# ltinphan/convex-mpc-unitree-go2

Measured on AMD Instinct MI355X. Metric: batched QP solves/sec (N=16, 4-leg friction cone) at 1/2/4/8 MI355X, higher is better.
Workload: dtype f32

## Files before the change

### convex-mpc-unitree-go2_amd/cmpc/_lib.py

```python
from __future__ import annotations

import ctypes
import os
from pathlib import Path

from .build import LIB

ABI_VERSION = 6
ABI_COMPAT = (5, 6) if os.environ.get("CMPC_ALLOW_ABI5") == "1" else (6,)
NUM_STATS = 4
CMPC_OK = 0


class CParams(ctypes.Structure):
    _fields_ = [
        ("abi_version", ctypes.c_int32),
        ("N", ctypes.c_int32),
        ("Q", ctypes.c_float * 12),
        ("R", ctypes.c_float * 12),
        ("mu", ctypes.c_float),
        ("fz_min", ctypes.c_float),
        ("eps_abs", ctypes.c_float),
        ("eps_rel", ctypes.c_float),
        ("max_iter", ctypes.c_int32),
# ... 5 lines not shown
        ("polish_refine", ctypes.c_int32),
        ("polish_tol", ctypes.c_float),
        ("polish_repairs", ctypes.c_int32),
        ("reserved0", ctypes.c_int32),
        ("check_termination", ctypes.c_int32),
        ("max_batch", ctypes.c_int64),
    ]


def _io_fields(*names):
    head = ("Ad", "Bd", "gd", "x0", "xref", "contact", "mu", "fz_min")
    values = dict(face_tol=ctypes.c_float, prim_tol=ctypes.c_float, dual_tol=ctypes.c_float,
                  max_rounds=ctypes.c_int32)
    return ([("size", ctypes.c_uint32)] +
            [(n, values.get(n, ctypes.c_void_p)) for n in head + names])


class CSolveIO(ctypes.Structure):
    _fields_ = _io_fields("w_init", "y_init", "lam_init", "w_out", "y_out", "lam_out", "status",
                          "iters", "Q", "R")


class CKktIO(ctypes.Structure):
    _fields_ = _io_fields("Q", "R", "w", "lam", "face_tol", "res")


class CGainIO(ctypes.Structure):
    _fields_ = _io_fields("Q", "R", "w", "faces", "face_tol", "K", "Vx", "Vxx", "u_star",
                          "faces_out")


class CVjpIO(ctypes.Structure):
    _fields_ = _io_fields("Q", "R", "w", "faces", "face_tol", "gw", "g_x0", "g_xref", "g_gd", "g_Q",
                          "g_R", "g_mu", "g_fz_min", "g_Ad", "g_Bd")


class CRefineIO(ctypes.Structure):
    _fields_ = _io_fields("Q", "R", "w", "faces", "face_tol", "max_rounds", "prim_tol", "dual_tol",
                          "info", "res", "w64", "lam_out", "faces_out", "w_out", "status")


REFINE_INVALID, REFINE_ROUNDS, REFINE_CYCLE, REFINE_MAX_ROUNDS = -1, -2, -3, 16
REFINE_OUTPUTS = ("info", "res", "w64", "lam", "faces")

FACE_FZ_MIN, FACE_FX_POS, FACE_FX_NEG, FACE_FY_POS, FACE_FY_NEG = 1, 2, 4, 8, 16
GAIN_OUTPUTS = ("K", "Vx", "Vxx", "u_star", "faces")
VJP_OUTPUTS = ("x0", "xref", "gd", "Q", "R", "mu", "fz_min", "Ad", "Bd")

KKT_COLUMNS = ("cost", "stat", "prim", "comp")

EXPORTS = ("cmpc_params_default", "cmpc_plan_create", "cmpc_solve", "cmpc_plan_destroy",
           "cmpc_build_dynamics", "cmpc_solve_warm", "cmpc_solve_ref", "cmpc_solve_io_run", "cmpc_kkt_run", "cmpc_gain_run", "cmpc_vjp_run", "cmpc_refine_run", "cmpc_generate_traj", "cmpc_leg_torque", "cmpc_srb_step",
           "cmpc_plan_set_timing", "cmpc_plan_timing_read", "cmpc_plan_set_team", "cmpc_plan_team_batch",
           "cmpc_plan_set_heavy_first",
           "cmpc_plan_heavy_first_batch", "cmpc_plan_solve_kernel", "cmpc_plan_stats",
           "cmpc_last_error", "cmpc_version")
NUM_BINS = 5
BIN_CAPS = (96, 128, 144, 160, 192)
NUM_SOLVE_KERNELS = 3
KERNEL_BINS = ((1, 0), (3, 2), (4,))
KERNEL_NAMES = ("solve_group_kernel<128, 96>", "solve_group_kernel<160, 144>",
                "solve_group_kernel<192, 0>")

_lib = None


def load(path: str | Path | None = None) -> ctypes.CDLL:
    global _lib
    if _lib is not None and path is None:
        return _lib
    if path is None and os.environ.get("CMPC_LIB"):
        path = os.environ["CMPC_LIB"]
    p = Path(path) if path is not None else LIB
    if not p.exists():
        raise RuntimeError(f"cmpc: HIP library {p} not built (run __graft_entry__.build() or "
                           f"python -m cmpc.build); there is no CPU fallback")
    lib = ctypes.CDLL(str(p))
    vp = ctypes.c_void_p
    lib.cmpc_params_default.argtypes = [ctypes.POINTER(CParams)]
    lib.cmpc_params_default.restype = None
    lib.cmpc_plan_create.argtypes = [ctypes.POINTER(CParams), ctypes.POINTER(vp)]
    lib.cmpc_plan_create.restype = ctypes.c_int
    lib.cmpc_solve.argtypes = [vp, ctypes.c_int64] + [vp] * 10
    lib.cmpc_solve.restype = ctypes.c_int
    if hasattr(lib, "cmpc_solve_warm"):
        lib.cmpc_solve_warm.argtypes = [vp, ctypes.c_int64] + [vp] * 13
        lib.cmpc_solve_warm.restype = ctypes.c_int
    if hasattr(lib, "cmpc_solve_ref"):
        lib.cmpc_solve_ref.argtypes = [vp, ctypes.c_int64] + [vp] * 13
        lib.cmpc_solve_ref.restype = ctypes.c_int
    if hasattr(lib, "cmpc_solve_io_run"):
        lib.cmpc_solve_io_run.argtypes = [vp, ctypes.c_int64, ctypes.POINTER(CSolveIO), vp]
        lib.cmpc_solve_io_run.restype = ctypes.c_int
    if hasattr(lib, "cmpc_kkt_run"):
        lib.cmpc_kkt_run.argtypes = [vp, ctypes.c_int64, ctypes.POINTER(CKktIO), vp]
        lib.cmpc_kkt_run.restype = ctypes.c_int
    if hasattr(lib, "cmpc_gain_run"):
        lib.cmpc_gain_run.argtypes = [vp, ctypes.c_int64, ctypes.POINTER(CGainIO), vp]
        lib.cmpc_gain_run.restype = ctypes.c_int
    if hasattr(lib, "cmpc_vjp_run"):
        lib.cmpc_vjp_run.argtypes = [vp, ctypes.c_int64, ctypes.POINTER(CVjpIO), vp]
        lib.cmpc_vjp_run.restype = ctypes.c_int
    if hasattr(lib, "cmpc_refine_run"):
        lib.cmpc_refine_run.argtypes = [vp, ctypes.c_int64, ctypes.POINTER(CRefineIO), vp]
        lib.cmpc_refine_run.restype = ctypes.c_int
    lib.cmpc_build_dynamics.argtypes = [vp, ctypes.c_int64, ctypes.c_float] + [vp] * 8
    lib.cmpc_build_dynamics.restype = ctypes.c_int
    if hasattr(lib, "cmpc_generate_traj"):
        lib.cmpc_generate_traj.argtypes = [vp, ctypes.c_int64, ctypes.c_double] + [vp] * 11
        lib.cmpc_generate_traj.restype = ctypes.c_int
    if hasattr(lib, "cmpc_leg_torque"):
        lib.cmpc_leg_torque.argtypes = ([vp, ctypes.c_int64, vp, vp, vp, ctypes.c_int64] +
                                        [vp] * 12 + [ctypes.c_double, vp, vp])
        lib.cmpc_leg_torque.restype = ctypes.c_int
    if hasattr(lib, "cmpc_srb_step"):
        lib.cmpc_srb_step.argtypes = ([vp, ctypes.c_int64, ctypes.c_int, ctypes.c_double] + [vp] * 5 +
                                      [ctypes.c_int64] + [vp] * 5)
        lib.cmpc_srb_step.restype = ctypes.c_int
    lib.cmpc_plan_destroy.argtypes = [vp]
    lib.cmpc_plan_destroy.restype = None
    lib.cmpc_plan_set_timing.argtypes = [vp, ctypes.c_int]
    lib.cmpc_plan_set_timing.restype = ctypes.c_int
    lib.cmpc_plan_timing_read.argtypes = [vp, ctypes.POINTER(ctypes.c_float),
                                          ctypes.POINTER(ctypes.c_int32)]
    lib.cmpc_plan_timing_read.restype = ctypes.c_int
    if hasattr(lib, "cmpc_plan_set_team"):
        lib.cmpc_plan_set_team.argtypes = [vp, ctypes.c_int64]
        lib.cmpc_plan_set_team.restype = ctypes.c_int
        lib.cmpc_plan_team_batch.argtypes = [vp, ctypes.POINTER(ctypes.c_int64)]
        lib.cmpc_plan_team_batch.restype = ctypes.c_int
    if hasattr(lib, "cmpc_plan_set_heavy_first"):
        lib.cmpc_plan_set_heavy_first.argtypes = [vp, ctypes.c_int64]
        lib.cmpc_plan_set_heavy_first.restype = ctypes.c_int
        lib.cmpc_plan_heavy_first_batch.argtypes = [vp, ctypes.POINTER(ctypes.c_int64)]
        lib.cmpc_plan_heavy_first_batch.restype = ctypes.c_int
    if hasattr(lib, "cmpc_plan_stats"):
        lib.cmpc_plan_stats.argtypes = [vp, ctypes.POINTER(ctypes.c_uint64), ctypes.c_int]
        lib.cmpc_plan_stats.restype = ctypes.c_int
    if hasattr(lib, "cmpc_plan_solve_kernel"):
        lib.cmpc_plan_solve_kernel.argtypes = [vp, ctypes.c_int64, ctypes.c_int]
        lib.cmpc_plan_solve_kernel.restype = ctypes.c_char_p
    lib.cmpc_last_error.argtypes = []
    lib.cmpc_last_error.restype = ctypes.c_char_p
    lib.cmpc_version.argtypes = []
    lib.cmpc_version.restype = ctypes.c_char_p
    if path is None:
        _lib = lib
    return lib


def last_error(lib=None) -> str:
    lib = lib or load()
    return lib.cmpc_last_error().decode()
```

### convex-mpc-unitree-go2_amd/cmpc/solver.py

```python
from __future__ import annotations

import ctypes
from dataclasses import dataclass, field, fields
from typing import Optional

import torch

from . import _lib

STATUS_STRINGS = {1: "solved", 2: "solved inaccurate", -2: "maximum iterations reached",
                  -10: "unsolved"}
KKT_COLUMNS = _lib.KKT_COLUMNS


@dataclass
class SolverParams:
    N: int = 16
    Q: tuple = (1, 1, 50, 10, 20, 1, 2, 2, 1, 1, 1, 1)
    R: tuple = (1e-5,) * 12
    mu: float = 0.8
    fz_min: float = 10.0
    eps_abs: float = 1e-4
    eps_rel: float = 1e-4
    max_iter: int = 1000
# ... 97 lines not shown
            self._h = None

    def __del__(self):
        try:
            self.close()
        except Exception:
            pass

    def _same_device(self, t: torch.Tensor):
        if t.device != self.device:
            raise ValueError(f"cmpc: tensors are on {t.device} but the plan was created on "
                             f"{self.device}")

    def _fill_io(self, io, required: dict, optional: dict):
        for spec, skip_none in ((required, False), (optional, True)):
            for name, (t, dtype, shape) in spec.items():
                if t is None and skip_none:
                    continue
                _dev_tensor(t, name, dtype, shape)
                self._same_device(t)
                setattr(io, name, t.data_ptr())

    def _need(self, entry: str, method: str):
        if not hasattr(self.lib, entry):
            raise CmpcError(f"cmpc: this libcmpc.so has no {entry}: Plan.{method} needs a library "
                            "built from sources that declare it")

    def _results(self, io, spec: dict, want, always, out, device) -> dict:
        out = dict(out or {})
        res = {}
        for name in tuple(always) + tuple(n for n in want if n not in always):
            field, dtype, shape = spec[name]
            t = out.get(name)
            if t is None:
                t = torch.empty(shape, dtype=dtype, device=device)
            _dev_tensor(t, name, dtype, shape)
            self._same_device(t)
            setattr(io, field, t.data_ptr())
            res[name] = t
        return res

    def set_timing(self, enable: bool):
        _check(self.lib, self.lib.cmpc_plan_set_timing(self._h, int(bool(enable))),
               "cmpc_plan_set_timing")

    def set_team(self, max_batch: int):
        _check(self.lib, self.lib.cmpc_plan_set_team(self._h, int(max_batch)),
               "cmpc_plan_set_team")

    def team_batch(self) -> int:
        v = ctypes.c_int64()
        _check(self.lib, self.lib.cmpc_plan_team_batch(self._h, ctypes.byref(v)),
               "cmpc_plan_team_batch")
        return int(v.value)

    def set_heavy_first(self, min_batch: int):
        _check(self.lib, self.lib.cmpc_plan_set_heavy_first(self._h, int(min_batch)),
               "cmpc_plan_set_heavy_first")

    def heavy_first_batch(self) -> int:
        v = ctypes.c_int64()
        _check(self.lib, self.lib.cmpc_plan_heavy_first_batch(self._h, ctypes.byref(v)),
               "cmpc_plan_heavy_first_batch")
        return int(v.value)

    def solve_kernels(self, B: int) -> list:
        if not hasattr(self.lib, "cmpc_plan_solve_kernel"):
            return [None] * _lib.NUM_SOLVE_KERNELS
        out = []
        for k in range(_lib.NUM_SOLVE_KERNELS):
            r = self.lib.cmpc_plan_solve_kernel(self._h, int(B), k)
            out.append(r.decode() if r else None)
        return out

    def stats(self, reset: bool = False) -> dict:
        keys = ("loose", "status2_cert", "guard_refactors", "reserved")
        if not hasattr(self.lib, "cmpc_plan_stats"):
            return {k: None for k in keys[:3]}
        v = (ctypes.c_uint64 * _lib.NUM_STATS)()
        _check(self.lib, self.lib.cmpc_plan_stats(self._h, v, int(bool(reset))), "cmpc_plan_stats")
        return {k: int(x) for k, x in zip(keys[:3], list(v))}

    def timing_read(self):
        ms = (ctypes.c_float * 4)()
        calls = (ctypes.c_int32 * 4)()
        _check(self.lib, self.lib.cmpc_plan_timing_read(self._h, ms, calls),
               "cmpc_plan_timing_read")
        k = _lib.NUM_SOLVE_KERNELS
        return list(ms)[:k], list(calls)[:k]

    def solve(self, Ad, Bd, gd, x0, xref, contact, out=None, stream=None, w_init=None,
              y_init=None, y_out=None, lam_init=None, lam_out=None, mu=None, fz_min=None,
              Q=None, R=None):
        N = self.params.N
        B = Ad.shape[0]
        f32 = torch.float32
        for name, spec in _problem_spec(B, N, Ad, Bd, gd, x0, xref, contact).items():
            _dev_tensor(spec[0], name, *spec[1:])
        self._same_device(Ad)
        for t in (Bd, gd, x0, xref, contact):
            if t.device != Ad.device:
                raise ValueError("all inputs must be on the same device")
        if out is None:
            w = torch.empty((B, 24 * N), dtype=f32, device=Ad.device)
            status = torch.empty((B,), dtype=torch.int32, device=Ad.device)
            iters = torch.empty((B,), dtype=torch.int32, device=Ad.device)
# ... 334 lines not shown
```

### convex-mpc-unitree-go2_amd/csrc/cmpc_device.h

```cpp
#pragma once
#include <stdint.h>

namespace cmpc {

struct KParams {
  int N;
  float Q2[12];
  float R2[12];
  float mu, fz_min;
  float rho0, sigma, alpha;
  float eps_abs, eps_rel;
  float polish_tol;
  float r2_min;
  int max_iter;
  int adaptive_interval;
  int polish_stable;
  int polish_refine;
  int polish_repairs;
  int check_every;
  int latency_mode;
};

struct Inputs {
  const float* Ad = nullptr;
  const float* Bd = nullptr;
  const float* gd = nullptr;
  const float* x0 = nullptr;
  const float* xref = nullptr;
  const uint8_t* contact = nullptr;
  const float* w_init = nullptr;
  const float* y_init = nullptr;
  const float* lam_init = nullptr;
  const float* mu = nullptr;
  const float* fz_min = nullptr;
  const float* Q = nullptr;
  const float* R = nullptr;
};
struct Outputs {
  float* w = nullptr;
  int32_t* status = nullptr;
  int32_t* iters = nullptr;
  float* y = nullptr;
  float* lam = nullptr;
  unsigned long long* stats = nullptr;
};

constexpr int kNumBins = 5;
constexpr int kBinCap[kNumBins] = {96, 128, 144, 160, 192};

}
```

### convex-mpc-unitree-go2_amd/csrc/cmpc_host.hip

```cpp
#include <hip/hip_runtime.h>
#include <stddef.h>
#include <stdlib.h>
#include <stdint.h>
#include <stdio.h>
#include <string.h>

#include <algorithm>
#include <cmath>
#include <string>
#include <vector>

#include "cmpc.h"
#include "cmpc_device.h"

#include "cmpc_wave.hip"
#include "cmpc_dynamics.hip"
#include "cmpc_traj.hip"
#include "cmpc_leg.hip"
#include "cmpc_sim.hip"
#include "cmpc_kkt.hip"
#include "cmpc_gain.hip"
#include "cmpc_vjp.hip"
#include "cmpc_refine.hip"

// ... 170 lines not shown
  p->max_batch = 65536;
}

int cmpc_plan_create(const cmpc_params* p, cmpc_plan** out) {
  if (!p || !out) return fail(CMPC_E_INVALID, "cmpc_plan_create: null argument");
  *out = nullptr;
  if (p->abi_version != CMPC_ABI_VERSION)
    return fail(CMPC_E_INVALID, "cmpc_plan_create: abi_version mismatch");
  if (p->N < 1 || p->N > 16) return fail(CMPC_E_INVALID, "cmpc_plan_create: N must be in 1..16");
  for (int i = 0; i < 12; ++i) {
    if (!(p->Q[i] >= 0.f) || !std::isfinite(p->Q[i]))
      return fail(CMPC_E_INVALID, "cmpc_plan_create: Q must be finite and >= 0");
    if (!(p->R[i] > 0.f) || !std::isfinite(p->R[i]))
      return fail(CMPC_E_INVALID, "cmpc_plan_create: R must be finite and > 0");
  }
  if (!(p->mu > 0.f) || !std::isfinite(p->mu)) return fail(CMPC_E_INVALID, "cmpc_plan_create: mu must be > 0");
  if (!std::isfinite(p->fz_min)) return fail(CMPC_E_INVALID, "cmpc_plan_create: fz_min must be finite");
  if (p->max_iter < 1) return fail(CMPC_E_INVALID, "cmpc_plan_create: max_iter must be >= 1");
  if (!(p->rho > 0.f) || !(p->sigma >= 0.f) || !(p->alpha > 0.f && p->alpha < 2.f))
    return fail(CMPC_E_INVALID, "cmpc_plan_create: need rho > 0, sigma >= 0, 0 < alpha < 2");
  if (p->polish_stable < 1 || p->polish_refine < 1 || !(p->polish_tol > 0.f) ||
      p->polish_repairs < 0 || p->check_termination < 1)
    return fail(CMPC_E_INVALID, "cmpc_plan_create: polish settings out of range");
  if (p->adaptive_rho_interval < 0 || p->max_batch < 1 || p->max_batch > (1LL << 30))
    return fail(CMPC_E_INVALID, "cmpc_plan_create: adaptive_rho_interval/max_batch out of range");
  if (p->reserved0 != 0)
    return fail(CMPC_E_INVALID, "cmpc_plan_create: reserved0 must be 0 (ABI 4's ipm_facts: the "
                                "interior-point fallback was removed)");

  cmpc_plan* pl = new cmpc_plan();
  pl->p = *p;
  cmpc::KParams& k = pl->kp;
  k.N = p->N;
  k.r2_min = 2.f * p->R[0];
  for (int i = 0; i < 12; ++i) {
    k.Q2[i] = 2.f * p->Q[i];
    k.R2[i] = 2.f * p->R[i];
    k.r2_min = std::min(k.r2_min, k.R2[i]);
  }
  k.mu = p->mu;
  k.fz_min = p->fz_min;
  k.rho0 = p->rho;
  k.sigma = p->sigma;
  k.alpha = p->alpha;
  k.eps_abs = p->eps_abs;
  k.eps_rel = p->eps_rel;
  k.polish_tol = p->polish_tol;
  k.max_iter = p->max_iter;
  k.adaptive_interval = p->adaptive_rho_interval;
  k.polish_stable = p->polish_stable;
  k.polish_refine = p->polish_refine;
  k.polish_repairs = p->polish_repairs;
  k.check_every = p->check_termination;

  hipError_t e = hipGetDevice(&pl->device);
  if (e != hipSuccess) { delete pl; return hip_fail(e, "hipGetDevice"); }
  int cus = 0;
  e = hipDeviceGetAttribute(&cus, hipDeviceAttributeMultiprocessorCount, pl->device);
  pl->cus = cus;
  if (e != hipSuccess) { delete pl; return hip_fail(e, "hipDeviceGetAttribute"); }
  size_t work_floats = 0;
  for (int k = 0; k < kNumGroups; ++k) {
    int nb = 0;
    e = hipOccupancyMaxActiveBlocksPerMultiprocessor(&nb, group_fn(k), 64, 0);
    if (e != hipSuccess) { delete pl; return hip_fail(e, "hipOccupancyMaxActiveBlocksPerMultiprocessor"); }
    if (nb < 1) { delete pl; return fail(CMPC_E_HIP, "cmpc_plan_create: solve kernel cannot be resident"); }
#ifdef CMPC_STAMPS
    if (const char* cap = getenv("CMPC_BLOCKS_PER_CU")) {
      const int c = atoi(cap);
      if (c >= 1 && c < nb) nb = c;
    }
#endif
    pl->grid[k] = nb * cus;
    pl->slab[k] = group_slab(k);
    pl->work_off[k] = work_floats;
    work_floats += (size_t)pl->grid[k] * pl->slab[k];
  }
  {
    int nb = 0;
    e = hipOccupancyMaxActiveBlocksPerMultiprocessor(&nb, cmpc::solve_team_kernel<kTeamWaves, 2>,
                                                     64 * kTeamWaves, 0);
    if (e != hipSuccess) { delete pl; return hip_fail(e, "hipOccupancyMaxActiveBlocksPerMultiprocessor"); }
    if (nb < 1) nb = 1;
    pl->team_grid = nb * cus;
    e = hipOccupancyMaxActiveBlocksPerMultiprocessor(&nb, cmpc::solve_team_kernel<kTeamWaves, 1>,
                                                     64 * kTeamWaves, 0);
    if (e != hipSuccess) { delete pl; return hip_fail(e, "hipOccupancyMaxActiveBlocksPerMultiprocessor"); }
    pl->team_grid1 = nb < 1 ? 0 : cus;
    pl->team_slab = std::max({cmpc::TeamCfg<192, kTeamWaves>::SLAB, cmpc::TeamCfg<160, kTeamWaves>::SLAB,
                              cmpc::TeamCfg<128, kTeamWaves>::SLAB, cmpc::TeamCfg<96, kTeamWaves>::SLAB});
    work_floats = std::max(work_floats, (size_t)pl->team_grid * pl->team_slab);
  }
  e = hipMalloc(&pl->d_counters, 2 * cmpc::kNumBins * sizeof(int));
  if (e != hipSuccess) { delete pl; return fail(CMPC_E_NOMEM, "hipMalloc counters failed"); }
  e = hipMalloc(&pl->d_work, work_floats * sizeof(float));
  if (e != hipSuccess) {
    (void)hipFree(pl->d_counters);
    delete pl;
    return fail(CMPC_E_NOMEM, "hipMalloc workspace failed");
  }
  e = hipMalloc(&pl->d_lists, (size_t)cmpc::kNumBins * p->max_batch * sizeof(int));
  if (e != hipSuccess) {
    (void)hipFree(pl->d_counters);
    (void)hipFree(pl->d_work);
    delete pl;
    return fail(CMPC_E_NOMEM, "hipMalloc lists failed");
// ... 372 lines not shown
  if (B == 0) return CMPC_OK;
  if (!t || !gait || !force || !J_foot || !J_full || !M || !C || !g || !dq || !Jdot_dq ||
      !foot_pos || !foot_vel || !body || !hip || !state || !tau)
    return fail(CMPC_E_INVALID, "cmpc_leg_torque: null array argument");
  cmpc::LegArgs a{t, gait, force, force_stride, J_foot, J_full, M, C, g, dq, Jdot_dq, foot_pos,
                  foot_vel, body, hip, state, tau_max, tau};
  hipLaunchKernelGGL(cmpc::leg_kernel, dim3(grid_stride_blocks(B, 16384)), dim3(64), 0,
                     (hipStream_t)stream, B, a);
  hipError_t e = hipGetLastError();
  if (e != hipSuccess) return hip_fail(e, "leg_kernel launch");
  return CMPC_OK;
}

int cmpc_srb_step(cmpc_plan* pl, int64_t B, int nsub, double dt, const double* t_now,
                  const double* gait, const float* mass, const float* inertia_body,
                  const float* force, int64_t force_stride, const float* hip, float* x,
                  float* feet, uint8_t* contact_state, void* stream) {
  if (!pl) return fail(CMPC_E_INVALID, "cmpc_srb_step: null plan");
  if (int rc = check_device(pl, "cmpc_srb_step")) return rc;
  if (B < 0 || nsub < 0) return fail(CMPC_E_INVALID, "cmpc_srb_step: negative batch or nsub");
  if (!(dt > 0.0) || !std::isfinite(dt)) return fail(CMPC_E_INVALID, "cmpc_srb_step: dt must be > 0");
  if (force_stride < 12) return fail(CMPC_E_INVALID, "cmpc_srb_step: force_stride must be >= 12");
  if (B == 0 || nsub == 0) return CMPC_OK;
  if (!t_now || !gait || !mass || !inertia_body || !force || !hip || !x || !feet || !contact_state)
    return fail(CMPC_E_INVALID, "cmpc_srb_step: null array argument");
  const unsigned blocks = (unsigned)((B + 255) / 256);
  hipLaunchKernelGGL(cmpc::srb_kernel, dim3(blocks), dim3(256), 0, (hipStream_t)stream, B, nsub,
                     dt, t_now, gait, mass, inertia_body, force, force_stride, hip, x, feet,
                     contact_state);
  hipError_t e = hipGetLastError();
  if (e != hipSuccess) return hip_fail(e, "srb_kernel launch");
  return CMPC_OK;
}

int cmpc_plan_set_timing(cmpc_plan* pl, int enable) {
  if (!pl) return fail(CMPC_E_INVALID, "cmpc_plan_set_timing: null plan");
  pl->timing = enable != 0;
  return CMPC_OK;
}

int cmpc_plan_set_team(cmpc_plan* pl, int64_t max_batch) {
  if (!pl) return fail(CMPC_E_INVALID, "cmpc_plan_set_team: null plan");
  if (max_batch < -1) return fail(CMPC_E_INVALID, "cmpc_plan_set_team: max_batch must be >= -1");
  pl->team_max_batch = max_batch;
  return CMPC_OK;
}

int cmpc_plan_team_batch(const cmpc_plan* pl, int64_t* max_batch) {
  if (!pl || !max_batch) return fail(CMPC_E_INVALID, "cmpc_plan_team_batch: null argument");
  *max_batch = team_batch(pl);
  return CMPC_OK;
}

int cmpc_plan_set_heavy_first(cmpc_plan* pl, int64_t min_batch) {
  if (!pl) return fail(CMPC_E_INVALID, "cmpc_plan_set_heavy_first: null plan");
  if (min_batch < -1) return fail(CMPC_E_INVALID, "cmpc_plan_set_heavy_first: min_batch must be >= -1");
  pl->heavy_first_min_batch = min_batch;
  return CMPC_OK;
}

int cmpc_plan_heavy_first_batch(const cmpc_plan* pl, int64_t* min_batch) {
  if (!pl || !min_batch) return fail(CMPC_E_INVALID, "cmpc_plan_heavy_first_batch: null argument");
  *min_batch = heavy_first_batch(pl);
  return CMPC_OK;
}

const char* cmpc_plan_solve_kernel(const cmpc_plan* pl, int64_t B, int k) {
  if (!pl || B < 1 || k < 0 || k >= kNumGroups) return nullptr;
  if (B <= team_batch(pl))
    return k != 0 ? nullptr : team_one_per_cu(pl, B) ? "solve_team_kernel<4, 1>" : "solve_team_kernel<4, 2>";
  if (!has_group(pl, k)) return nullptr;
  return group_name(k);
}

int cmpc_plan_timing_read(cmpc_plan* pl, float* ms_per_kernel, int32_t* calls_per_kernel) {
  if (!pl || !ms_per_kernel || !calls_per_kernel)
    return fail(CMPC_E_INVALID, "cmpc_plan_timing_read: null argument");
  for (int k = 0; k < kNumGroups; ++k) { ms_per_kernel[k] = 0.f; calls_per_kernel[k] = 0; }
  for (auto& r : pl->recs) {
    hipError_t e = hipEventSynchronize(r.b);
    if (e != hipSuccess) return hip_fail(e, "hipEventSynchronize");
    float ms = 0.f;
    e = hipEventElapsedTime(&ms, r.a, r.b);
    if (e != hipSuccess) return hip_fail(e, "hipEventElapsedTime");
    ms_per_kernel[r.group] += ms;
    calls_per_kernel[r.group] += 1;
    pl->pool.push_back(r);
  }
  pl->recs.clear();
  return CMPC_OK;
}

void cmpc_plan_destroy(cmpc_plan* pl) {
  if (!pl) return;
  for (auto& r : pl->recs) { (void)hipEventDestroy(r.a); (void)hipEventDestroy(r.b); }
  for (auto& r : pl->pool) { (void)hipEventDestroy(r.a); (void)hipEventDestroy(r.b); }
  if (pl->side) (void)hipStreamDestroy(pl->side);
  if (pl->top) (void)hipStreamDestroy(pl->top);
  if (pl->fork) (void)hipEventDestroy(pl->fork);
  if (pl->join) (void)hipEventDestroy(pl->join);
  if (pl->join_top) (void)hipEventDestroy(pl->join_top);
  (void)hipFree(pl->d_counters);
  (void)hipFree(pl->d_lists);
  (void)hipFree(pl->d_work);
  if (pl->d_stats) (void)hipFree(pl->d_stats);
  delete pl;
// ... 33 lines not shown
```

### convex-mpc-unitree-go2_amd/csrc/cmpc_solve.h

```cpp
#pragma once
#include "cmpc_team.hip"

#include "cmpc_condense.h"
#include "cmpc_factor.h"
#include "cmpc_gradient.h"
#include "cmpc_polish.h"

namespace cmpc {

template <int NC>
__device__ __forceinline__ int session_start(Smem<NC>& s, const KParams& P, int ntri, int nfail,
                                             int& ntried, bool& seen) {
  const int l = opaque_lane();
  WSYNC();
  uint8_t c = 0;
  if (l < ntri) {
    c = (uint8_t)s.code[l];
    s.tpat[0][l] = c;
  }
  ntried = 1;
  seen = false;
#pragma unroll
  for (int k = 0; k < kFailMem; ++k) {
    if (k >= nfail) break;
    const bool diff = (l < ntri) && (s.fpat[k][l] != c);
    seen |= (__any(diff) == 0);
  }
  if (seen) return 0;
  return (nfail >= 2) ? min(P.polish_repairs, kLateRepairs) : P.polish_repairs;
}

template <int NC>
__device__ __forceinline__ bool tried_before(Smem<NC>& s, int ntri, int ntried) {
  const int l = opaque_lane();
  WSYNC();
  const uint8_t c = (l < ntri) ? (uint8_t)s.tcnt[l] : 0;
  bool hit = false;
  for (int k = 0; k < ntried; ++k) {
    const bool diff = (l < ntri) && (s.tpat[k][l] != c);
    hit |= (__any(diff) == 0);
  }
  return hit;
}


template <int NC>
constexpr bool kRhoLow = (NC == 128) || (kRhoLowHeavy && NC > 128);

struct Instance {
  int64_t b;
  int N, NP;
  Terrain T;
  bool weights_ok;
  float r2_min;
  const float* Bg;
  const float* xrb;
  int ntri, n;
  bool nil;
  const f4* pwc;
  const f4* twc;
};

struct Ctl {
  int status = -2, iters = 0;
  bool polished = false;
  float rp = 0.f, rd = 0.f, np_ = 0.f, nd = 0.f;
  float rho = 0.f;
  bool rho_low = false;
  int stable = 0;
  bool refactor = false;
  bool in_polish = false;
  int nact = 0;
  float shift = 0.f;
  int it = 0;
  int repairs_left = 0;
  int nadd = 0;
  bool from_cand = false;
  bool parked = false;
  int nfail = 0;
  int ntried = 0;
  bool seen_start = false;
  int last_pol = 0;
  bool fail_rho_done = false;
  bool warm_session = false;
};

__device__ __forceinline__ void set_rho(Ctl& c, const KParams& P, float rho, bool low) {
  c.rho = rho;
  c.rho_low = low;
  c.shift = uniformf(P.sigma + c.rho);
  c.refactor = true;
}

template <int NC>
__device__ __forceinline__ void stage_instance(Smem<NC>& s, const KParams& P, const Inputs& in,
                                               Instance& I, int lane) {
  const int64_t b = I.b;
  const int N = I.N, NP = I.NP;
  const Terrain T = I.T;
  bool weights_ok = true;
  float r2_min = P.r2_min;
  const float* Ab = in.Ad + b * 144;
  const float* Bg = in.Bd + b * (int64_t)N * 144;
  const float* gdb = in.gd + b * 12;
  const float* x0b = in.x0 + b * 12;
  const float* xrb = in.xref + b * (int64_t)N * 12;
  const uint8_t* ctb = in.contact + b * (int64_t)4 * N;

  WSYNC();
  const uint8_t ctv = (lane < 4 * N) ? ctb[(lane & 3) * N + (lane >> 2)] : (uint8_t)0;
  float bw[36];
  if (lane < 4 * N) {
    const float* src = Bg + lane * 36;
#pragma unroll
    for (int i = 0; i < 36; ++i) bw[i] = src[i];
  } else {
#pragma unroll
    for (int i = 0; i < 36; ++i) bw[i] = 0.f;
  }
  {
    float av[3], rv[4];
#pragma unroll
    for (int i = 0; i < 3; ++i) {
      const int e = lane + 64 * i;
      av[i] = (e < 144) ? Ab[e] : 0.f;
    }
#pragma unroll
    for (int i = 0; i < 4; ++i) {
      const int e = lane + 64 * i;
      rv[i] = (e < 12) ? x0b[e] : (e < 12 * (N + 1)) ? xrb[e - 12] : 0.f;
    }
    const float gv = (lane < 12) ? gdb[lane] : 0.f;
    if (in.Q || in.R) {
      const float q = (in.Q && lane < 12) ? in.Q[b * 12 + lane] : 0.f;
      const float r = (in.R && lane < 12) ? in.R[b * 12 + lane] : 1.f;
      weights_ok = __any(!(q >= 0.f && isfinite(q) && r > 0.f && isfinite(r))) == 0;
      if (lane < 12) {
// ... 104 lines not shown
  CMPC_CNT(8, 1);
  TRACEF(I.b, "it %d FACTOR polish %d nact %d shift %g\n", c.it, (int)c.in_polish, c.nact, c.shift);
  diag.factor();
  if constexpr (W == 1) {
    CMPC_T0(t_c);
    condense_tiles<NC>(s, P, M, c.nact, uniformf(c.shift), I.nil);
    CMPC_ACC(0, t_c);
    CMPC_T0(t_i);
    ldl_tiles<NC>(s, M, c.nact);
    CMPC_ACC(1, t_i);
  } else {
    CMPC_T0(t_c);
    team_factor_lead<NC, W>(s, *ts, *seq, P, M, c.nact, uniformf(c.shift));
    CMPC_ACC(0, t_c);
  }
  c.refactor = false;
}

template <int NC, int W>
__device__ __forceinline__ void apply_factors(Smem<NC>& s, TeamSmem<NC, W>* ts, int* seq,
                                              const f4 (&M)[TeamCfg<NC, W>::SLOTS], int n,
                                              const float* in, float* out) {
  if constexpr (W == 1) ldl_apply<NC>(s, M, n, in, out);
  else team_symv_lead<NC, W>(s, *ts, *seq, M, n, in, out);
}

template <int NC, int W>
__device__ __forceinline__ void park_tiles(float* __restrict__ park, TeamSmem<NC, W>* ts, int* seq,
                                           const f4 (&M)[TeamCfg<NC, W>::SLOTS]) {
  if constexpr (W == 1) {
    park_store<NC>(park, M);
  } else {
    team_issue<NC, W>(*ts, *seq, kOpParkStore, 0, 0, 0);
    team_park_store<NC, W, 0>(park, M, 0);
  }
}

template <int NC, int W>
__device__ __forceinline__ void restore_tiles(const float* __restrict__ park, TeamSmem<NC, W>* ts,
                                              int* seq, f4 (&M)[TeamCfg<NC, W>::SLOTS]) {
  if constexpr (W == 1) {
    park_load<NC>(park, M);
  } else {
    team_issue<NC, W>(*ts, *seq, kOpParkLoad, 0, 0, 0);
    team_park_load<NC, W, 0>(park, M, 0);
  }
}

template <int NC>
__device__ __forceinline__ void enter_polish(Smem<NC>& s, const KParams& P, const Instance& I,
                                             Ctl& c) {
  c.repairs_left = session_start<NC>(s, P, I.ntri, c.nfail, c.ntried, c.seen_start);
  c.nact = polish_setup<NC>(s, P, I.T, I.Bg, I.ntri, s.z);
  c.nadd = 0;
  c.shift = P.sigma;
  c.refactor = true;
  c.in_polish = true;
}

template <int NC>
__device__ __forceinline__ void refactor_faces(Smem<NC>& s, const KParams& P, const Instance& I,
                                               Ctl& c, const float* from) {
  c.nact = polish_setup<NC>(s, P, I.T, I.Bg, I.ntri, from);
  c.nadd = 0;
  c.shift = P.sigma;
  c.refactor = true;
}

struct Refined {
  float step, vscale;
  bool stalled;
  PolishCheck chk;
};

template <int NC, int W>
__device__ __forceinline__ Refined polish_refine(Smem<NC>& s, const KParams& P, const Instance& I,
                                                 Ctl& c, f4 (&M)[TeamCfg<NC, W>::SLOTS],
                                                 TeamSmem<NC, W>* ts, int* seq, int lane) {
  Refined r;
  r.step = 3.0e38f;
  r.vscale = 1.f;
  r.stalled = false;
  float prev = 3.0e38f;
  const int nact = c.nact;
  const int qmin = c.from_cand ? 1 : P.polish_refine;
  c.from_cand = false;
  for (int pass = 0;; ++pass) {
    for (int q = pass == 0 ? 0 : P.polish_refine + kRefineExtra - 1;
         q < P.polish_refine + kRefineExtra; ++q) {
      gradient<NC, kGradLat<NC, W>, true>(s, P, nact, s.v, s.g, I.pwc, I.twc);
      apply_factors<NC, W>(s, ts, seq, M, nact, s.g, s.dl);
      if constexpr (W == 1) {
        if (c.nadd > 0) dd_apply<NC>(s, nact, c.nadd, s.g, s.dl);
      }
      float m = 0.f, mv = 1.f;
      for (int p = lane; p < nact; p += 64) {
        const float vn = s.v[p] - s.dl[p];
        s.v[p] = vn;
        m = fmaxf(m, fabsf(s.dl[p]));
        mv = fmaxf(mv, fabsf(vn));
      }
      r.step = wave_max(m);
      r.vscale = wave_max(mv);
      TRACEF(I.b, "    refine %d step %g\n", q, r.step);
      r.stalled = r.step > kRefineRate * prev;
      if (q + 1 >= qmin && (r.step <= P.polish_tol * wave_max(mv) || r.stalled)) break;
      prev = r.step;
    }
    gradient<NC, kGradLat<NC, W>, true>(s, P, nact, s.v, s.g, I.pwc, I.twc);
    const int top = (kRepairTop > 0 && (c.nfail > 0 || c.ntried >= 3)) ? kRepairTop : 0;
    r.chk = polish_check<NC>(s, P, I.T, I.Bg, I.ntri, r.step, top, trace_id(I.b));
    if (!(r.chk.amb && (r.chk.ok || r.chk.loose)) || pass >= kAmbRefine ||
        r.step <= kAmbConverged * P.polish_tol * r.vscale)
      break;
  }
  return r;
// ... 125 lines not shown
  c.nact = I.n;
  c.nadd = 0;
  set_rho(c, P, kRhoLow<NC> ? 0.5f * P.rho0 : P.rho0, kRhoLow<NC>);
  c.stable = 0;
  c.last_pol = 0;
  c.ntried = 0;
  c.seen_start = false;
  c.parked = false;
}

template <int NC, int W>
__device__ __forceinline__ void session_failed(Smem<NC>& s, const KParams& P, const Instance& I,
                                               Ctl& c, f4 (&M)[TeamCfg<NC, W>::SLOTS],
                                               float* __restrict__ park, TeamSmem<NC, W>* ts,
                                               int* seq, Diag& diag, int lane) {
  c.warm_session = false;
  TRACEF(I.b, "it %d SESSION-FAIL nfail %d seen %d parked %d rho_low %d fail_rho_done %d nadd %d\n",
         c.it, c.nfail, (int)c.seen_start, (int)c.parked, (int)c.rho_low, (int)c.fail_rho_done,
         c.nadd);
  diag.session_failed();
  if (!c.seen_start) {
    const int l = opaque_lane();
    if (l < I.ntri) s.fpat[c.nfail % kFailMem][l] = s.tpat[0][l];
    ++c.nfail;
  }
  build_admm_basis<NC>(s, P, I.Bg, I.ntri);
  c.in_polish = false;
  c.nact = I.n;
  if (c.nfail == 1 && !c.seen_start && kFailRho != 1.f && !c.fail_rho_done) {
    c.fail_rho_done = true;
    set_rho(c, P, uniformf(kFailRho * P.rho0), false);
    return;
  }
  if (c.rho_low) {
    set_rho(c, P, uniformf(P.rho0), false);
    return;
  }
  c.shift = uniformf(P.sigma + c.rho);
  if (c.parked) {
    restore_tiles<NC, W>(park, ts, seq, M);
  } else {
    c.refactor = true;
  }
}

template <int NC, int W>
__device__ __forceinline__ bool admm_iteration(Smem<NC>& s, const KParams& P, const Instance& I,
                                               Ctl& c, const f4 (&M)[TeamCfg<NC, W>::SLOTS],
                                               TeamSmem<NC, W>* ts, int* seq, int lane) {
  const int n = I.n, ntri = I.ntri, it = c.it;
  const Terrain T = I.T;
  const float alpha = P.alpha;
  float rho = c.rho;
  gradient<NC, kGradLat<NC, W>>(s, P, n, s.x, s.g, I.pwc, I.twc);
  {
    const int l = opaque_lane();
    if (l < ntri) {
#pragma unroll
      for (int a = 0; a < 3; ++a) {
        const int p = 3 * l + a;
        s.r[p] = rho * (s.z[p] - s.x[p]) - s.g[p] - s.y[p];
      }
    }
  }
  apply_factors<NC, W>(s, ts, seq, M, n, s.r, s.dl);
  CMPC_T0(t_rest);
  const bool last = (it == P.max_iter);
  const bool adapt = P.adaptive_interval > 0 && (it % P.adaptive_interval) == 0;
  const float inv_rho = 1.f / rho;
  float lrp = 0.f, lrd = 0.f, lnp = 0.f, lnd = 0.f;
  bool changed = false;
  {
    const int l = opaque_lane();
    if (l < ntri) {
      float w[3], xr[3], xs[3];
#pragma unroll
      for (int a = 0; a < 3; ++a) {
        const int p = 3 * l + a;
        const float x = s.x[p], z = s.z[p];
        const float xt = x + s.dl[p];
        xr[a] = alpha * xt + (1.f - alpha) * z;
        xs[a] = alpha * xt + (1.f - alpha) * x;
        w[a] = xr[a] + s.y[p] * inv_rho;
      }
      float pv[3];
      const int code = project(w[0], w[1], w[2], T.mu, T.fz_min, pv[0], pv[1], pv[2]);
#pragma unroll
      for (int a = 0; a < 3; ++a) {
        const int p = 3 * l + a;
        const float zn = pv[a];
        const float yn = s.y[p] + rho * (xr[a] - zn);
        s.x[p] = xs[a];
        s.z[p] = zn;
        s.y[p] = yn;
        const float gp = s.g[p];
        lrp = fmaxf(lrp, fabsf(xs[a] - zn));
        lrd = fmaxf(lrd, fabsf(gp + yn));
        lnp = fmaxf(lnp, fmaxf(fabsf(xs[a]), fabsf(zn)));
        lnd = fmaxf(lnd, fmaxf(fabsf(gp), fabsf(yn)));
      }
      changed = code != s.pcode[l];
      s.pcode[l] = code;
      s.code[l] = code;
    }
  }
  if (trace_on(I.b)) {
    const float trp = wave_max(lrp), trd = wave_max(lrd);
    TRACEF(I.b, "it %d rho %g rp %g rd %g stable %d\n", it, rho, trp, trd, c.stable);
  }
  c.stable = (__any(changed) != 0) ? 0 : c.stable + 1;
  bool do_pol = false;
  const int pstable = P.polish_stable;
  const int backoff = pstable << min(c.nfail, kBackoffCap);
  int need = pstable;
  for (int f = 0; f < min(c.nfail, kBackoffCap); ++f) need *= kStableGrow;
  if (c.stable >= need && !last && it - c.last_pol >= backoff &&
      (P.check_every == 1 || it % P.check_every == 0)) {
    do_pol = true;
    c.last_pol = it;
    c.stable = -backoff;
  }
  if (adapt || last) {
    c.rp = wave_max(lrp); c.rd = wave_max(lrd); c.np_ = wave_max(lnp); c.nd = wave_max(lnd);
  }
  if (adapt && !last) {
    float q = rho * sqrtf((c.rp / fmaxf(c.np_, 1e-30f)) / (c.rd / fmaxf(c.nd, 1e-30f) + 1e-30f));
    q = fminf(fmaxf(q, 1e-6f), 1e6f);
    if (q > 5.f * rho || q < 0.2f * rho) set_rho(c, P, uniformf(q), false);
  }
  CMPC_ACC(7, t_rest);
  return do_pol;
}

template <int NC, int W>
__device__ __forceinline__ void start_session(Smem<NC>& s, const KParams& P, const Instance& I,
                                              Ctl& c, const f4 (&M)[TeamCfg<NC, W>::SLOTS],
                                              float* __restrict__ park, TeamSmem<NC, W>* ts,
                                              int* seq, Diag& diag, int lane) {
  CMPC_CNT(9, 1);
  diag.polish_attempt();
  CMPC_T0(t_ps);
  const bool pending = c.refactor;
  c.parked = !c.refactor && !c.rho_low && c.nfail > 0;
  if (c.parked) park_tiles<NC, W>(park, ts, seq, M);
  enter_polish<NC>(s, P, I, c);
  TRACEF(I.b, "it %d SESSION nfail %d parked %d rho %g refactor_pending %d seen %d repairs %d nact %d\n",
         c.it, c.nfail, (int)c.parked, c.rho, (int)pending, (int)c.seen_start, c.repairs_left,
         c.nact);
  CMPC_ACC(14, t_ps);
}

template <int NC>
__device__ __forceinline__ int force_triple(const Smem<NC>& s, int o, int& a) {
  const int k = o / 12, l = (o % 12) / 3;
  a = o % 3;
  return s.tri_of[4 * k + l];
}

template <int NC>
__device__ __forceinline__ bool write_w(Smem<NC>& s, const Instance& I, float* wb, bool polished,
                                        int lane) {
  const int NP = I.NP;
  const float* uf = polished ? s.x : s.z;
  int bad = 0;
  for (int o = lane; o < NP; o += 64) {
    const float xv = s.E[o] + I.xrb[o];
    int a;
    const int t = force_triple(s, o, a);
    const float uv = (t >= 0) ? uf[3 * t + a] : 0.f;
    bad |= !(isfinite(xv) && isfinite(uv));
    wb[o] = xv;
    wb[NP + o] = uv;
  }
  return __any(bad) == 0;
}

template <int NC, int W>
__device__ __forceinline__ void write_y(Smem<NC>& s, const KParams& P, const Instance& I,
                                        float* yb, bool polished, int lane) {
// ... 25 lines not shown
  for (int o = lane; o < NP; o += 64) {
    lb[o] = 0.f;
    lb[24 * N + o] = -s.L[o];
  }
  if (lane < 4 * N) {
    const int k = lane >> 2, leg = lane & 3;
    const int t = s.tri_of[lane];
    const float* Bk = I.Bg + k * 144 + 3 * leg;
    float sv[3], u[3];
#pragma unroll
    for (int a = 0; a < 3; ++a) {
      u[a] = (t >= 0) ? uf[3 * t + a] : 0.f;
      float acc = s.R2[3 * leg + a] * u[a];
#pragma unroll
      for (int r = 0; r < 12; ++r) acc = fmaf(Bk[r * 12 + a], s.L[12 * k + r], acc);
      sv[a] = acc;
    }
    float lf[4] = {0.f, 0.f, 0.f, 0.f}, lxv[3] = {0.f, 0.f, 0.f};
    if (t < 0) {
#pragma unroll
      for (int a = 0; a < 3; ++a) lxv[a] = -sv[a];
    } else {
      const int code = polished ? s.code[t]
                                : faces_at(u[0], u[1], u[2], T.mu, T.fz_min, 1e-5f * fmaxf(u[2], 1.f));
      if (code & 2) lf[0] = fmaxf(-sv[0], 0.f);
      if (code & 4) lf[1] = fmaxf(sv[0], 0.f);
      if (code & 8) lf[2] = fmaxf(-sv[1], 0.f);
      if (code & 16) lf[3] = fmaxf(sv[1], 0.f);
      if (code & 1) lxv[2] = fminf(-(sv[2] - T.mu * (lf[0] + lf[1] + lf[2] + lf[3])), 0.f);
    }
    float* lxo = lb + NP + 12 * k + 3 * leg;
#pragma unroll
    for (int a = 0; a < 3; ++a) lxo[a] = lxv[a];
    float* lfo = lb + 24 * N + NP + 16 * k + 4 * leg;
#pragma unroll
    for (int f = 0; f < 4; ++f) lfo[f] = lf[f];
  }
}

template <int NC, int W>
__device__ __forceinline__ void solve_instance(Smem<NC>& s, const KParams& P, int64_t b,
                                               const Inputs& in, const Outputs& out,
                                               float* __restrict__ park, TeamSmem<NC, W>* ts,
                                               int* seq) {
  f4 M[TeamCfg<NC, W>::SLOTS];
  static_assert(W > 1 || TeamCfg<NC, W>::SLOTS == Cfg<NC>::NTL, "W = 1 holds every tile");
  const int lane = opaque_lane();
  Diag diag;
  Instance I;
  I.b = b;
  I.N = P.N;
  I.NP = 12 * P.N;
  I.T = instance_terrain(P, in, b);
  diag.poison(W == 1, s.G, 12 * NC, s.v, NC, park, Cfg<NC>::SLAB, lane);
  CMPC_T0(t_inst);
  CMPC_CNT(10, 1);
  stage_instance<NC>(s, P, in, I, lane);
  constexpr bool kPow = W > 1 && NC <= 128;
  f4 pw_c[4], tw_c[4];
  if constexpr (kPow) gradient_powers(s, pw_c, tw_c);
  I.pwc = kPow ? pw_c : nullptr;
  I.twc = kPow ? tw_c : nullptr;
  const int n = I.n;

  Ctl c;
  set_rho(c, P, kRhoLow<NC> ? 0.5f * P.rho0 : P.rho0, kRhoLow<NC>);
  starting_point<NC>(s, in, I, c.rho, lane);
  CMPC_ACC(6, t_inst);
  diag.begin();
  c.refactor = n > 0;
  c.nact = n;
  if (n == 0) c.status = 1;
  if (n > 0 && in.w_init != nullptr) {
    c.warm_session = true;
    WSYNC();
    if (lane < I.ntri) s.code[lane] = s.pcode[lane];
    enter_polish<NC>(s, P, I, c);
  }
  while (n > 0) {
    if (c.refactor) factorize<NC, W>(s, P, I, c, M, ts, seq, diag, lane);
    if (c.in_polish) {
      switch (polish_pass<NC, W>(s, P, I, out, c, M, ts, seq, diag, lane)) {
        case Polish::kAccepted: accept_point<NC>(s, I, out, c, diag, lane); break;
        case Polish::kAcceptedLoose: accept_loose<NC>(s, I, out, c, diag, lane); break;
        case Polish::kRefactorSameSet: refactor_faces<NC>(s, P, I, c, s.dl); continue;
        case Polish::kRepaired: repair_faces<NC, W>(s, P, I, c, M, lane); continue;
        case Polish::kWarmRestart: warm_restart<NC>(s, P, I, c); continue;
        case Polish::kSessionFailed:
          session_failed<NC, W>(s, P, I, c, M, park, ts, seq, diag, lane);
          if (c.refactor) continue;
          break;
      }
      if (c.polished) break;
    }
    if (c.it >= P.max_iter) break;
    c.iters = ++c.it;
    if (admm_iteration<NC, W>(s, P, I, c, M, ts, seq, lane))
      start_session<NC, W>(s, P, I, c, M, park, ts, seq, diag, lane);
  }
  if (!c.polished) {
    if (n > 0) {
      const bool conv = c.rp <= P.eps_abs + P.eps_rel * c.np_ && c.rd <= P.eps_abs + P.eps_rel * c.nd;
      c.status = conv ? 2 : -2;
    }
    gradient<NC, kGradLat<NC, W>>(s, P, n, s.z, s.g, I.pwc, I.twc);
  }
  TRACEF(b, "END status %d iters %d\n", c.status, c.iters);
  CMPC_T0(t_out);
  WSYNC();
  float* wb = out.w + b * (int64_t)(24 * I.N);
  if (!write_w<NC>(s, I, wb, c.polished, lane) || !terrain_valid(I.T) || !I.weights_ok)
    c.status = -10;
  if (out.y) write_y<NC, W>(s, P, I, out.y + b * (int64_t)I.NP, c.polished, lane);
  if (out.lam) write_lam<NC>(s, I, out.lam + b * (int64_t)(52 * I.N), c.polished, lane);
  diag.finish(out.status, out.iters, wb, b, lane, c.status, c.iters);
  CMPC_CNT(11, c.iters);
  CMPC_ACC(15, t_out);
  CMPC_ACC(5, t_inst);
}

template <int NC, int W>
__device__ __forceinline__ void drain_bin(Smem<NC>& s, const KParams& P, const Inputs& in,
                                          const Outputs& out, const int* __restrict__ list,
                                          const int* __restrict__ count, int* __restrict__ head,
                                          float* __restrict__ park, TeamSmem<NC, W>* ts = nullptr,
                                          int* seq = nullptr) {
  const int lane = opaque_lane();
  WSYNC();
  if (lane < 12) {
    s.Q2[lane] = P.Q2[lane];
    s.R2[lane] = P.R2[lane];
  }
  const int total = *count;
  for (;;) {
    int idx = 0;
    if (lane == 0) idx = atomicAdd(head, 1);
    idx = __builtin_amdgcn_readfirstlane(idx);
    if (idx >= total) break;
    const int64_t b = list[idx];
    solve_instance<NC, W>(s, P, b, in, out, park, ts, seq);
  }
  if constexpr (W > 1) team_issue<NC, W>(*ts, *seq, kOpExit, 0, 0, 0);
}

}
```

### include/cmpc.h

```cpp
#ifndef CMPC_H_
#define CMPC_H_

#include <stdint.h>

#ifdef __cplusplus
extern "C" {
#endif

#define CMPC_ABI_VERSION 6

#define CMPC_OK 0
#define CMPC_E_INVALID (-22)
#define CMPC_E_NOMEM (-12)
#define CMPC_E_HIP (-5)
#define CMPC_E_RANGE (-34)

typedef struct cmpc_params {
  int32_t abi_version;
  int32_t N;
  float Q[12];
  float R[12];
  float mu;
  float fz_min;
  float eps_abs;
// ... 117 lines not shown
  const float *mu, *fz_min;
  const float *Q, *R;
  const float* w;
  const uint8_t* faces;
  float face_tol;
  int32_t max_rounds;
  float prim_tol, dual_tol;
  int32_t* info;
  double* res;
  double* w64;
  double* lam_out;
  uint8_t* faces_out;
  float* w_out;
  int32_t* status;
} cmpc_refine_io;

#define CMPC_REFINE_INVALID (-1)
#define CMPC_REFINE_ROUNDS (-2)
#define CMPC_REFINE_CYCLE (-3)
#define CMPC_REFINE_MAX_ROUNDS 16
int cmpc_refine_run(cmpc_plan* plan, int64_t B, const cmpc_refine_io* io, void* stream);

void cmpc_plan_destroy(cmpc_plan* plan);

int cmpc_build_dynamics(cmpc_plan* plan, int64_t B, float dt, const float* mass,
                        const float* inertia, const float* r_feet, const float* xref,
                        float* Ad, float* Bd, float* gd, void* stream);

int cmpc_generate_traj(cmpc_plan* plan, int64_t B, double dt, const float* x0, double* pos_des,
                       const float* cmd, const double* t_now, const double* gait,
                       const float* foot_lever, const float* hip, float* xref, uint8_t* contact,
                       float* r_feet, void* stream);

int cmpc_leg_torque(cmpc_plan* plan, int64_t B, const double* t, const double* gait,
                    const float* force, int64_t force_stride, const double* J_foot,
                    const double* J_full, const double* M, const double* C, const double* g,
                    const double* dq, const double* Jdot_dq, const double* foot_pos,
                    const double* foot_vel, const double* body, const double* hip,
                    double* state, double tau_max, double* tau, void* stream);

int cmpc_srb_step(cmpc_plan* plan, int64_t B, int nsub, double dt, const double* t_now,
                  const double* gait, const float* mass, const float* inertia_body,
                  const float* force, int64_t force_stride, const float* hip, float* x,
                  float* feet, uint8_t* contact_state, void* stream);

#define CMPC_NUM_SOLVE_KERNELS 3
int cmpc_plan_set_timing(cmpc_plan* plan, int enable);
int cmpc_plan_timing_read(cmpc_plan* plan, float* ms_per_kernel, int32_t* calls_per_kernel);
const char* cmpc_plan_solve_kernel(const cmpc_plan* plan, int64_t B, int k);

int cmpc_plan_set_team(cmpc_plan* plan, int64_t max_batch);
int cmpc_plan_team_batch(const cmpc_plan* plan, int64_t* max_batch);

int cmpc_plan_set_heavy_first(cmpc_plan* plan, int64_t min_batch);
int cmpc_plan_heavy_first_batch(const cmpc_plan* plan, int64_t* min_batch);

#define CMPC_NUM_STATS 4
int cmpc_plan_stats(cmpc_plan* plan, uint64_t* out, int reset);

const char* cmpc_last_error(void);

const char* cmpc_version(void);

#ifdef __cplusplus
}
#endif

#endif
```

Baseline: 8.705 million.

## Skip per-iteration QP gradient by using cached linear term in ADMM x-update

The ADMM x-update right-hand side is rewritten to use a cached linear cost term q (computed once as the gradient at zero) plus sigma*x, so the full Hessian-vector gradient is skipped on most iterations. The exact gradient path is still taken on adaptive-rho, final, failure, or optional periodic iterations, where residuals are needed. Residual bookkeeping is made local, with a stored convergence flag replacing the cached norms. This removes a matrix-vector product per iteration at the cost of extra branching and some floating-point drift from the algebraically equivalent form.

```diff
diff --git a/convex-mpc-unitree-go2_amd/cmpc/_lib.py b/convex-mpc-unitree-go2_amd/cmpc/_lib.py
--- a/convex-mpc-unitree-go2_amd/cmpc/_lib.py
+++ b/convex-mpc-unitree-go2_amd/cmpc/_lib.py
@@ -81,7 +81,7 @@
 EXPORTS = ("cmpc_params_default", "cmpc_plan_create", "cmpc_solve", "cmpc_plan_destroy",
            "cmpc_build_dynamics", "cmpc_solve_warm", "cmpc_solve_ref", "cmpc_solve_io_run", "cmpc_kkt_run", "cmpc_gain_run", "cmpc_vjp_run", "cmpc_refine_run", "cmpc_generate_traj", "cmpc_leg_torque", "cmpc_srb_step",
            "cmpc_plan_set_timing", "cmpc_plan_timing_read", "cmpc_plan_set_team", "cmpc_plan_team_batch",
-           "cmpc_plan_set_heavy_first",
+           "cmpc_plan_set_heavy_first", "cmpc_plan_set_admm_exact", "cmpc_plan_admm_exact",
            "cmpc_plan_heavy_first_batch", "cmpc_plan_solve_kernel", "cmpc_plan_stats",
            "cmpc_last_error", "cmpc_version")
 NUM_BINS = 5
@@ -158,6 +158,11 @@
         lib.cmpc_plan_set_team.restype = ctypes.c_int
         lib.cmpc_plan_team_batch.argtypes = [vp, ctypes.POINTER(ctypes.c_int64)]
         lib.cmpc_plan_team_batch.restype = ctypes.c_int
+    if hasattr(lib, "cmpc_plan_set_admm_exact"):
+        lib.cmpc_plan_set_admm_exact.argtypes = [vp, ctypes.c_int]
+        lib.cmpc_plan_set_admm_exact.restype = ctypes.c_int
+        lib.cmpc_plan_admm_exact.argtypes = [vp, ctypes.POINTER(ctypes.c_int)]
+        lib.cmpc_plan_admm_exact.restype = ctypes.c_int
     if hasattr(lib, "cmpc_plan_set_heavy_first"):
         lib.cmpc_plan_set_heavy_first.argtypes = [vp, ctypes.c_int64]
         lib.cmpc_plan_set_heavy_first.restype = ctypes.c_int
diff --git a/convex-mpc-unitree-go2_amd/cmpc/solver.py b/convex-mpc-unitree-go2_amd/cmpc/solver.py
--- a/convex-mpc-unitree-go2_amd/cmpc/solver.py
+++ b/convex-mpc-unitree-go2_amd/cmpc/solver.py
@@ -173,6 +173,18 @@
         v = ctypes.c_int64()
         _check(self.lib, self.lib.cmpc_plan_team_batch(self._h, ctypes.byref(v)),
                "cmpc_plan_team_batch")
+        return int(v.value)
+
+    def set_admm_exact(self, every: int):
+        self._need("cmpc_plan_set_admm_exact", "set_admm_exact")
+        _check(self.lib, self.lib.cmpc_plan_set_admm_exact(self._h, int(every)),
+               "cmpc_plan_set_admm_exact")
+
+    def admm_exact(self) -> int:
+        self._need("cmpc_plan_admm_exact", "admm_exact")
+        v = ctypes.c_int()
+        _check(self.lib, self.lib.cmpc_plan_admm_exact(self._h, ctypes.byref(v)),
+               "cmpc_plan_admm_exact")
         return int(v.value)
 
     def set_heavy_first(self, min_batch: int):
diff --git a/convex-mpc-unitree-go2_amd/csrc/cmpc_device.h b/convex-mpc-unitree-go2_amd/csrc/cmpc_device.h
--- a/convex-mpc-unitree-go2_amd/csrc/cmpc_device.h
+++ b/convex-mpc-unitree-go2_amd/csrc/cmpc_device.h
@@ -18,6 +18,7 @@
   int polish_refine;
   int polish_repairs;
   int check_every;
+  int admm_exact;
   int latency_mode;
 };
 
diff --git a/convex-mpc-unitree-go2_amd/csrc/cmpc_host.hip b/convex-mpc-unitree-go2_amd/csrc/cmpc_host.hip
--- a/convex-mpc-unitree-go2_amd/csrc/cmpc_host.hip
+++ b/convex-mpc-unitree-go2_amd/csrc/cmpc_host.hip
@@ -246,6 +246,7 @@
   k.polish_refine = p->polish_refine;
   k.polish_repairs = p->polish_repairs;
   k.check_every = p->check_termination;
+  k.admm_exact = 0;
 
   hipError_t e = hipGetDevice(&pl->device);
   if (e != hipSuccess) { delete pl; return hip_fail(e, "hipGetDevice"); }
@@ -724,6 +725,19 @@
   return CMPC_OK;
 }
 
+int cmpc_plan_set_admm_exact(cmpc_plan* pl, int every) {
+  if (!pl) return fail(CMPC_E_INVALID, "cmpc_plan_set_admm_exact: null plan");
+  if (every < 0) return fail(CMPC_E_INVALID, "cmpc_plan_set_admm_exact: every must be >= 0");
+  pl->kp.admm_exact = every;
+  return CMPC_OK;
+}
+
+int cmpc_plan_admm_exact(const cmpc_plan* pl, int* every) {
+  if (!pl || !every) return fail(CMPC_E_INVALID, "cmpc_plan_admm_exact: null argument");
+  *every = pl->kp.admm_exact;
+  return CMPC_OK;
+}
+
 int cmpc_plan_set_heavy_first(cmpc_plan* pl, int64_t min_batch) {
   if (!pl) return fail(CMPC_E_INVALID, "cmpc_plan_set_heavy_first: null plan");
   if (min_batch < -1) return fail(CMPC_E_INVALID, "cmpc_plan_set_heavy_first: min_batch must be >= -1");
diff --git a/convex-mpc-unitree-go2_amd/csrc/cmpc_solve.h b/convex-mpc-unitree-go2_amd/csrc/cmpc_solve.h
--- a/convex-mpc-unitree-go2_amd/csrc/cmpc_solve.h
+++ b/convex-mpc-unitree-go2_amd/csrc/cmpc_solve.h
@@ -57,6 +57,7 @@
   const float* xrb;
   int ntri, n;
   bool nil;
+  bool dual_start;
   const f4* pwc;
   const f4* twc;
 };
@@ -64,7 +65,7 @@
 struct Ctl {
   int status = -2, iters = 0;
   bool polished = false;
-  float rp = 0.f, rd = 0.f, np_ = 0.f, nd = 0.f;
+  bool conv = true;
   float rho = 0.f;
   bool rho_low = false;
   int stable = 0;
@@ -83,6 +84,7 @@
   int last_pol = 0;
   bool fail_rho_done = false;
   bool warm_session = false;
+  bool q_valid = false;
 };
 
 __device__ __forceinline__ void set_rho(Ctl& c, const KParams& P, float rho, bool low) {
@@ -293,6 +295,7 @@
                                              Ctl& c) {
   c.repairs_left = session_start<NC>(s, P, I.ntri, c.nfail, c.ntried, c.seen_start);
   c.nact = polish_setup<NC>(s, P, I.T, I.Bg, I.ntri, s.z);
+  c.q_valid = false;
   c.nadd = 0;
   c.shift = P.sigma;
   c.refactor = true;
@@ -303,6 +306,7 @@
 __device__ __forceinline__ void refactor_faces(Smem<NC>& s, const KParams& P, const Instance& I,
                                                Ctl& c, const float* from) {
   c.nact = polish_setup<NC>(s, P, I.T, I.Bg, I.ntri, from);
+  c.q_valid = false;
   c.nadd = 0;
   c.shift = P.sigma;
   c.refactor = true;
@@ -534,21 +538,51 @@
   const Terrain T = I.T;
   const float alpha = P.alpha;
   float rho = c.rho;
-  gradient<NC, kGradLat<NC, W>>(s, P, n, s.x, s.g, I.pwc, I.twc);
+  const bool last = (it == P.max_iter);
+  const bool adapt = P.adaptive_interval > 0 && (it % P.adaptive_interval) == 0;
+  const bool copy_q = !c.q_valid && it == 1 && !I.dual_start;
+  const bool exact = copy_q || adapt || last || c.nfail > 0 ||
+                     (P.admm_exact > 0 && it % P.admm_exact == 0);
+  const bool make_q = !c.q_valid && !exact;
+  if (make_q) {
+    const int l = opaque_lane();
+    for (int p = l; p < n; p += 64) {
+      s.r[p] = s.x[p];
+      s.x[p] = 0.f;
+    }
+  }
+  if (exact || make_q)
+    gradient<NC, kGradLat<NC, W>>(s, P, n, s.x, s.g, I.pwc, I.twc);
+  if (copy_q || make_q) {
+    const int l = opaque_lane();
+    for (int p = l; p < n; p += 64) {
+      s.v[p] = s.g[p];
+      if (make_q) s.x[p] = s.r[p];
+    }
+    c.q_valid = true;
+    WSYNC();
+  }
   {
     const int l = opaque_lane();
     if (l < ntri) {
 #pragma unroll
       for (int a = 0; a < 3; ++a) {
         const int p = 3 * l + a;
-        s.r[p] = rho * (s.z[p] - s.x[p]) - s.g[p] - s.y[p];
+        if (exact) s.r[p] = rho * (s.z[p] - s.x[p]) - s.g[p] - s.y[p];
+        else s.r[p] = fmaf(P.sigma, s.x[p], rho * s.z[p]) - s.y[p] - s.v[p];
       }
     }
   }
   apply_factors<NC, W>(s, ts, seq, M, n, s.r, s.dl);
+  if (!exact) {
+    const int l = opaque_lane();
+    WSYNC();
+    if (l < ntri) {
+#pragma unroll
+      for (int a = 0; a < 3; ++a) s.dl[3 * l + a] -= s.x[3 * l + a];
+    }
+  }
   CMPC_T0(t_rest);
-  const bool last = (it == P.max_iter);
-  const bool adapt = P.adaptive_interval > 0 && (it % P.adaptive_interval) == 0;
   const float inv_rho = 1.f / rho;
   float lrp = 0.f, lrd = 0.f, lnp = 0.f, lnd = 0.f;
   bool changed = false;
@@ -575,11 +609,13 @@
         s.x[p] = xs[a];
         s.z[p] = zn;
         s.y[p] = yn;
-        const float gp = s.g[p];
-        lrp = fmaxf(lrp, fabsf(xs[a] - zn));
-        lrd = fmaxf(lrd, fabsf(gp + yn));
-        lnp = fmaxf(lnp, fmaxf(fabsf(xs[a]), fabsf(zn)));
-        lnd = fmaxf(lnd, fmaxf(fabsf(gp), fabsf(yn)));
+        if (exact) {
+          const float gp = s.g[p];
+          lrp = fmaxf(lrp, fabsf(xs[a] - zn));
+          lrd = fmaxf(lrd, fabsf(gp + yn));
+          lnp = fmaxf(lnp, fmaxf(fabsf(xs[a]), fabsf(zn)));
+          lnd = fmaxf(lnd, fmaxf(fabsf(gp), fabsf(yn)));
+        }
       }
       changed = code != s.pcode[l];
       s.pcode[l] = code;
@@ -602,11 +638,13 @@
     c.last_pol = it;
     c.stable = -backoff;
   }
+  float rp = 0.f, rd = 0.f, np_ = 0.f, nd = 0.f;
   if (adapt || last) {
-    c.rp = wave_max(lrp); c.rd = wave_max(lrd); c.np_ = wave_max(lnp); c.nd = wave_max(lnd);
+    rp = wave_max(lrp); rd = wave_max(lrd); np_ = wave_max(lnp); nd = wave_max(lnd);
+    c.conv = rp <= P.eps_abs + P.eps_rel * np_ && rd <= P.eps_abs + P.eps_rel * nd;
   }
   if (adapt && !last) {
-    float q = rho * sqrtf((c.rp / fmaxf(c.np_, 1e-30f)) / (c.rd / fmaxf(c.nd, 1e-30f) + 1e-30f));
+    float q = rho * sqrtf((rp / fmaxf(np_, 1e-30f)) / (rd / fmaxf(nd, 1e-30f) + 1e-30f));
     q = fminf(fmaxf(q, 1e-6f), 1e6f);
     if (q > 5.f * rho || q < 0.2f * rho) set_rho(c, P, uniformf(q), false);
   }
@@ -738,6 +776,7 @@
   I.N = P.N;
   I.NP = 12 * P.N;
   I.T = instance_terrain(P, in, b);
+  I.dual_start = in.w_init == nullptr && (in.y_init != nullptr || in.lam_init != nullptr);
   diag.poison(W == 1, s.G, 12 * NC, s.v, NC, park, Cfg<NC>::SLAB, lane);
   CMPC_T0(t_inst);
   CMPC_CNT(10, 1);
@@ -750,6 +789,7 @@
   const int n = I.n;
 
   Ctl c;
+  c.conv = 0.f <= P.eps_abs + P.eps_rel * 0.f;
   set_rho(c, P, kRhoLow<NC> ? 0.5f * P.rho0 : P.rho0, kRhoLow<NC>);
   starting_point<NC>(s, in, I, c.rho, lane);
   CMPC_ACC(6, t_inst);
@@ -786,8 +826,7 @@
   }
   if (!c.polished) {
     if (n > 0) {
-      const bool conv = c.rp <= P.eps_abs + P.eps_rel * c.np_ && c.rd <= P.eps_abs + P.eps_rel * c.nd;
-      c.status = conv ? 2 : -2;
+      c.status = c.conv ? 2 : -2;
     }
     gradient<NC, kGradLat<NC, W>>(s, P, n, s.z, s.g, I.pwc, I.twc);
   }
diff --git a/include/cmpc.h b/include/cmpc.h
--- a/include/cmpc.h
+++ b/include/cmpc.h
@@ -193,6 +193,9 @@
 int cmpc_plan_set_team(cmpc_plan* plan, int64_t max_batch);
 int cmpc_plan_team_batch(const cmpc_plan* plan, int64_t* max_batch);
 
+int cmpc_plan_set_admm_exact(cmpc_plan* plan, int every);
+int cmpc_plan_admm_exact(const cmpc_plan* plan, int* every);
+
 int cmpc_plan_set_heavy_first(cmpc_plan* plan, int64_t min_batch);
 int cmpc_plan_heavy_first_batch(const cmpc_plan* plan, int64_t* min_batch);
 
```

Result: no change. 8.783 million (median of 6 runs) (+0.9%).
